# tatsuya-ogawa/metal4-raytracing

Hardware: AMD Instinct MI355X
Metric: Grays/sec (closest-hit + shadow rays traced) at 1920x1080x4spp, dragon; ms/frame (higher is better)
Workload: dtype f32; 1 GPU; c3g: glass dragon scene (configs[2]) 1920x1080x4spp, 8 bounces, one frame per step, single GPU, frames submitted back to back (overlapping frames in flight); scene=c3g, triangles=881218, width=1920, height=1080, spp=4, max_bounces=8, pipeline=wavefront, parallelism=tiles1, rays_per_frame=31537269, sort_bins=0, bvh=sah, frames_in_flight=8, animate=False

## Files before the change

metal4-raytracing_amd/csrc/rt_wavefront.hip:

```cpp
#include "rt_shade.h"
#include "rt_wavefront.h"

#include <array>
#include <utility>

namespace rt {

namespace {

__device__ __forceinline__ uint32_t lane_id() { return __builtin_amdgcn_mbcnt_hi(~0u, __builtin_amdgcn_mbcnt_lo(~0u, 0u)); }
__device__ __forceinline__ uint32_t mbcnt64(unsigned long long m) {
    return __builtin_amdgcn_mbcnt_hi((uint32_t)(m >> 32), __builtin_amdgcn_mbcnt_lo((uint32_t)m, 0u));
}

struct BlockAlloc {
    uint32_t w[kBlock / 64];
};

__device__ __forceinline__ uint32_t block_alloc(bool pred, uint32_t* counter, BlockAlloc& sh) {
    const int wave = threadIdx.x >> 6;
    unsigned long long m = __ballot(pred);
    uint32_t prefix = mbcnt64(m);
    if (lane_id() == 0) sh.w[wave] = (uint32_t)__popcll(m);
    __syncthreads();
    if (threadIdx.x == 0) {
        uint32_t c0 = sh.w[0], c1 = sh.w[1], c2 = sh.w[2], c3 = sh.w[3];
        uint32_t tot = c0 + c1 + c2 + c3;
        uint32_t b = tot ? atomicAdd(counter, tot) : 0u;
        sh.w[0] = b;
        sh.w[1] = b + c0;
        sh.w[2] = b + c0 + c1;
        sh.w[3] = b + c0 + c1 + c2;
    }
    __syncthreads();
    uint32_t r = sh.w[wave] + prefix;
    __syncthreads();
    return r;
}

struct BlockAllocOct {
    uint32_t cnt[3][8];
    uint32_t base[3][8];
};
__device__ __forceinline__ void block_alloc3_oct(const bool (&pr)[3], uint32_t oct, uint32_t* const (&ctr)[3],
                                                 BlockAllocOct& sh, uint32_t (&out)[3]) {
    if (threadIdx.x < 24) (&sh.cnt[0][0])[threadIdx.x] = 0u;
    __syncthreads();
    uint32_t rank[3] = {0u, 0u, 0u};
    #pragma unroll
    for (int i = 0; i < 3; ++i)
        if (pr[i]) rank[i] = atomicAdd(&sh.cnt[i][i ? oct : 0u], 1u);
    __syncthreads();
    if (threadIdx.x < 3) {
        const int i = threadIdx.x;
        uint32_t tot = 0, pre[8];
        #pragma unroll
        for (int o = 0; o < 8; ++o) { pre[o] = tot; tot += sh.cnt[i][o]; }
        const uint32_t b = tot ? atomicAdd(ctr[i], tot) : 0u;
        #pragma unroll
        for (int o = 0; o < 8; ++o) sh.base[i][o] = b + pre[o];
    }
    __syncthreads();
    #pragma unroll
    for (int i = 0; i < 3; ++i) out[i] = sh.base[i][i ? oct : 0u] + rank[i];
    __syncthreads();
}

__device__ __forceinline__ uint32_t block_alloc_n(uint32_t v, uint32_t* counter, BlockAlloc& sh) {
    const int wave = threadIdx.x >> 6;
    const uint32_t lane = lane_id();
    uint32_t incl = v;
    #pragma unroll
    for (int off = 1; off < 64; off <<= 1) {
        uint32_t t = __shfl_up(incl, off, 64);
        if (lane >= (uint32_t)off) incl += t;
    }
    if (lane == 63) sh.w[wave] = incl;
    __syncthreads();
    if (threadIdx.x == 0) {
        uint32_t c0 = sh.w[0], c1 = sh.w[1], c2 = sh.w[2], c3 = sh.w[3];
        uint32_t tot = c0 + c1 + c2 + c3;
        uint32_t b = tot ? atomicAdd(counter, tot) : 0u;
        sh.w[0] = b;
        sh.w[1] = b + c0;
        sh.w[2] = b + c0 + c1;
        sh.w[3] = b + c0 + c1 + c2;
    }
    __syncthreads();
    uint32_t r = sh.w[wave] + incl - v;
    __syncthreads();
    return r;
}

__device__ __forceinline__ uint32_t wave_incl_scan(uint32_t v) {
    const uint32_t lane = lane_id();
    #pragma unroll
    for (int off = 1; off < 64; off <<= 1) {
        const uint32_t t = __shfl_up(v, off, 64);
        if (lane >= (uint32_t)off) v += t;
    }
    return v;
}

__device__ __forceinline__ uint32_t compact1by1(uint32_t x) {
    x &= 0x55555555u;
    x = (x | (x >> 1)) & 0x33333333u;
    x = (x | (x >> 2)) & 0x0f0f0f0fu;
    x = (x | (x >> 4)) & 0x00ff00ffu;
    x = (x | (x >> 8)) & 0x0000ffffu;
    return x;
}


__device__ __forceinline__ uint32_t pack_state(int bounce, int tpass, int step) {
    return (uint32_t)bounce | ((uint32_t)tpass << 8) | ((uint32_t)step << 16);
}

__device__ __forceinline__ uint32_t fdiv(uint32_t n, const FastDiv& f) {
    const uint32_t t = __umulhi(f.m, n);
    return (t + ((n - t) >> f.s1)) >> f.s2;
}

__device__ __forceinline__ void own_pixel(const WfParams& Q, uint32_t i, int& px, int& py) {
    const uint32_t T = (uint32_t)Q.tile;
    const uint32_t k = fdiv(i, Q.tile_px_div), r = i - k * Q.tile_px_div.d;
    const uint32_t tid = (uint32_t)Q.rank + k * (uint32_t)Q.nranks;
    const uint32_t ty = fdiv(tid, Q.tiles_x_div), tx = tid - ty * Q.tiles_x_div.d;
    uint32_t lx, ly;
    if ((T & (T - 1)) == 0) {
        lx = compact1by1(r);
        ly = compact1by1(r >> 1);
    } else {
        lx = r % T;
        ly = r / T;
    }
    px = (int)(tx * T + lx);
    py = (int)(ty * T + ly);
}

constexpr int kCntSorted = 26;
constexpr uint32_t kNoKey = 0xffffffffu;

__device__ __forceinline__ void ts_start(const WfParams& Q, int ts) {
    if (ts >= 0 && blockIdx.x == 0 && threadIdx.x == 0) Q.W.tstamp[ts * kTsStride] = __builtin_amdgcn_s_memrealtime();
}
__device__ __forceinline__ void ts_end(const WfParams& Q, int ts, uint32_t* done) {
    if (ts < 0 || lane_id() != 0) return;
    if (atomicAdd(done, 1u) == (blockDim.x + 63u) / 64u - 1u)
        atomicMax(&Q.W.tstamp[ts * kTsStride + kTsLine * (1 + (int)(blockIdx.x % 8u))],
                  (unsigned long long)__builtin_amdgcn_s_memrealtime());
}

__device__ __forceinline__ void stat_add(const WfParams& Q, int word, uint32_t v) {
    if (blockIdx.x == 0 && threadIdx.x == 0) atomicAdd(&Q.W.counts[kWfStat + word], v);
}
__device__ __forceinline__ bool tail_mode(const WfParams& Q) {
    return Q.dev_ctl && __builtin_amdgcn_readfirstlane(Q.W.counts[cslot(kCntTailMode)]) != 0u;
}

struct ShardPrefix {
    uint32_t end[kShards];
};
__device__ __forceinline__ ShardPrefix load_prefix(const uint32_t* cnt, uint32_t cap = 0xffffffffu) {
    ShardPrefix p;
    uint32_t acc = 0;
    #pragma unroll
    for (int k = 0; k < kShards; ++k) {
        acc += min(__builtin_amdgcn_readfirstlane(cnt[cslot(k)]), cap);
        p.end[k] = acc;
    }
    return p;
}
struct QueueShards {
    uint32_t L[kShards], S[kShards];
};
__device__ __forceinline__ QueueShards load_queue(const uint32_t* counts, int q, uint32_t seg_cap) {
    QueueShards r;
    #pragma unroll
    for (int k = 0; k < kShards; ++k) {
        const uint32_t l = min(__builtin_amdgcn_readfirstlane(counts[cslot(q * kShards + k)]), seg_cap);
        r.L[k] = l;
        r.S[k] = min(__builtin_amdgcn_readfirstlane(counts[cslot(kCntBack + q * kShards + k)]), seg_cap - l);
    }
    return r;
}
__device__ __forceinline__ uint32_t queue_len(const QueueShards& qs) {
    uint32_t n = 0;
    #pragma unroll
    for (int k = 0; k < kShards; ++k) n += qs.L[k] + qs.S[k];
    return n;
}
__device__ __forceinline__ uint32_t seg_pos(uint32_t g, uint32_t l, uint32_t seg_cap) {
    return g < l ? g : seg_cap - 1u - (g - l);
}
__device__ __forceinline__ uint32_t dense_entry(const QueueShards& qs, uint32_t g, uint32_t seg_cap) {
    uint32_t ltot = 0;
    #pragma unroll
    for (int k = 0; k < kShards; ++k) ltot += qs.L[k];
    const bool back = g >= ltot;
    if (back) g -= ltot;
    uint32_t k = 0, start = 0, acc = 0;
    #pragma unroll
    for (int j = 0; j < kShards - 1; ++j) {
        acc += back ? qs.S[j] : qs.L[j];
        const bool past = g >= acc;
        k = past ? (uint32_t)(j + 1) : k;
        start = past ? acc : start;
    }
    const uint32_t i = g - start;
    return k * seg_cap + (back ? seg_cap - 1u - i : i);
}
__device__ __forceinline__ bool likely_long(const PathRegs& p) {
    return p.tpass > 0 || p.bounce < p.step;
}

__device__ __forceinline__ void init_path(const WfParams& Q, uint32_t pid, uint32_t pix, int sample, uint32_t hidx) {
    Q.W.p_accum[pid] = make_float4(0.0f, 0.0f, 0.0f, 0.0f);
    if (pid >= Q.base_paths) Q.W.p_meta[pid] = make_uint4(pix, (uint32_t)sample, 0u, hidx);
}


__device__ __forceinline__ void flush_counters(const FrameParams& P, uint32_t closest, uint32_t shadow, uint32_t paths,
                                               const TraceCounters& tc, bool count, bool overflow,
                                               bool trace_kernel = false) {
    block_flush_counters(P.counters, closest, shadow, count ? tc.nodes : 0u, count ? tc.tris : 0u, paths, overflow,
                         trace_kernel, count ? tc.lds_nodes : 0u);
}

__device__ __forceinline__ void write_pixel_outputs(const FrameParams& P, uint32_t pix, const StepResult& r, const Hit& h,
                                                    bool full) {
    if (r.primary) P.prim_hit[pix] = make_uint4(h.id, __float_as_uint(h.u), __float_as_uint(h.v), 0u);
    if (full && r.gbuf && P.gbuffer) {
        size_t plane = (size_t)P.U.width * P.U.height;
        P.gbuffer[pix] = r.g0;
        P.gbuffer[plane + pix] = r.g1;
        P.gbuffer[2 * plane + pix] = r.g2;
        P.gbuffer[3 * plane + pix] = r.g3;
    }
}

}

struct Trav {
    RaySetup R;
    float best, bu, bv, bdet;
    uint32_t best_id, g_base, g_hits, t_base, t_mask, t_valid;
    bool g_flip, hit_any;
    int sp;
};

__device__ __forceinline__ void trav_start(Trav& T, f3 o, f3 d, float tmax) {
    T.R = ray_setup(o, d);
    T.best = tmax;
    T.best_id = 0xffffffffu;
    T.bu = T.bv = 0.0f;
    T.bdet = 1.0f;
    T.g_base = 0;
    T.g_hits = 1;
    T.g_flip = false;
    T.t_mask = 0;
    T.sp = 0;
    T.hit_any = false;
}

__device__ __forceinline__ uint32_t next_node(Trav& T, int* stack, bool& overflow) {
    if (!T.g_hits) {
        --T.sp;
        const uint32_t ent = (uint32_t)stack[T.sp * kBlock];
        T.g_base = ent >> 9;
        T.g_flip = (ent >> 8) & 1u;
        T.g_hits = ent & 0xffu;
    }
    const int r = T.g_flip ? highest_bit(T.g_hits) : lowest_bit(T.g_hits);
    T.g_hits &= ~(1u << r);
    if (T.g_hits) {
        if (T.sp < kStackSize) {
            stack[T.sp * kBlock] = (int)pack_group(T.g_base, T.g_flip, T.g_hits);
            ++T.sp;
        } else {
            overflow = true;
        }
    }
    return T.g_base + (uint32_t)r;
}

template <bool COUNT>
__device__ __forceinline__ void node_step(const DevScene& S, Trav& T, int* stack, TraceCounters& tc, bool& overflow,
                                          float cull) {
    const uint32_t ni = next_node(T, stack, overflow);
    if (COUNT) tc.nodes++;
    const NodeWords w = load_node8(S.nodes8, ni);
    test_node8_words(w, T.R, 0.0f, fminf(cull, T.best), T.g_hits, T.t_mask, T.t_valid, T.g_base, T.t_base, T.g_flip);
}

template <bool COUNT>
__device__ __forceinline__ bool trav_step(const DevScene& S, Trav& T, bool any, int* stack, TraceCounters& tc,
                                          bool& overflow, float cull) {
    bool tdone = false;
    if (T.t_mask != 0u) {
        const int k0 = lowest_bit(T.t_mask);
        T.t_mask &= T.t_mask - 1u;
        const bool two = T.t_mask != 0u;
        const int k1 = two ? lowest_bit(T.t_mask) : k0;
        if (two) T.t_mask &= T.t_mask - 1u;
#ifdef RT_XP_STALE_BOUND
        const float stale_bound = fminf(cull, T.best);
#define RT_ISECT(a, b, c) intersect_rot(T.R.pre, T.R.o, a, b, c, 0.0f, stale_bound, &t, &u, &v, &dt)
#else
#define RT_ISECT(a, b, c) intersect_rot(T.R.pre, T.R.o, a, b, c, 0.0f, fminf(cull, T.best), &t, &u, &v, &dt)
#endif
        const uint32_t kz = (uint32_t)T.R.pre.kz;
        const uint32_t f0 = tri_slot(T.t_base, T.t_valid, k0) * (uint32_t)kTriFloats + kz;
        const uint32_t f1 = tri_slot(T.t_base, T.t_valid, k1) * (uint32_t)kTriFloats + kz;
        const f3 a0 = tri_window_at(S.tris, f0), a1 = tri_window_at(S.tris, f0 + 5u), a2 = tri_window_at(S.tris, f0 + 10u);
        const uint32_t ida = tri_id_at(S.tris, f0 - kz);
        const f3 b0 = tri_window_at(S.tris, f1), b1 = tri_window_at(S.tris, f1 + 5u), b2 = tri_window_at(S.tris, f1 + 10u);
        const uint32_t idb = tri_id_at(S.tris, f1 - kz);
        if (COUNT) tc.tris += two ? 2u : 1u;
        float t, u, v, dt;
        if (RT_ISECT(a0, a1, a2)) {
            const uint32_t id = ida;
            if (any) {
                T.hit_any = true;
                tdone = true;
            } else if (t < T.best || id < T.best_id) {
                T.best = t;
                T.best_id = id;
                T.bu = u;
                T.bdet = dt;
                T.bv = v;
            }
        }
        if (two && !tdone && RT_ISECT(b0, b1, b2)) {
            const uint32_t id = idb;
            if (any) {
                T.hit_any = true;
                tdone = true;
            } else if (t < T.best || id < T.best_id) {
                T.best = t;
                T.best_id = id;
                T.bu = u;
                T.bdet = dt;
                T.bv = v;
            }
        }
    }
    if (!tdone && T.t_mask == 0u && (T.g_hits != 0u || T.sp > 0)) node_step<COUNT>(S, T, stack, tc, overflow, cull);
    return tdone || (T.t_mask == 0u && T.g_hits == 0u && T.sp == 0);
#undef RT_ISECT
}

__device__ __forceinline__ uint32_t base_hidx(const FrameParams& P, int spp, uint32_t pix, int s) {
    const Uniforms& U = P.U;
    const int maxExtra = (U.enableMotionAdaptiveSampling != 0) ? max(U.motionSamplingMaxExtraSamples, 0) : 0;
    const int frameOffset = (int)U.frameIndex * (spp + maxExtra) + s;
    return (uint32_t)(int)(P.random[pix] + (unsigned)frameOffset);
}
__device__ __forceinline__ bool base_path(const FrameParams& P, const WfParams& Q, const ShadeTabs& halton, uint32_t pid,
                                          uint32_t& pix, int& s, uint32_t& hidx, f3& o, f3& d) {
    const Uniforms& U = P.U;
    const uint32_t i = fdiv(pid, Q.spp_div);
    s = (int)(pid - i * Q.spp_div.d);
    int px, py;
    own_pixel(Q, i, px, py);
    if (px >= U.width || py >= U.height) return false;
    pix = (uint32_t)py * (uint32_t)U.width + (uint32_t)px;
    hidx = base_hidx(P, Q.spp, pix, s);
    primary_ray(U, halton, px, py, (int)hidx, o, d);
    return true;
}
__device__ __forceinline__ uint3 path_meta(const FrameParams& P, const WfParams& Q, uint32_t pid) {
    if (pid >= Q.base_paths) {
        const uint4 m = Q.W.p_meta[pid];
        return make_uint3(m.x, m.y, m.w);
    }
    const uint32_t i = fdiv(pid, Q.spp_div);
    const int s = (int)(pid - i * Q.spp_div.d);
    int px, py;
    own_pixel(Q, i, px, py);
    const uint32_t pix = (uint32_t)py * (uint32_t)P.U.width + (uint32_t)px;
    return make_uint3(pix, (uint32_t)s, base_hidx(P, Q.spp, pix, s));
}
__device__ __forceinline__ void init_pixel(const FrameParams& P, uint32_t pix) {
    P.depth[pix] = 1.0e8f;
    P.motion[pix] = make_float2(0.0f, 0.0f);
    P.prim_hit[pix] = make_uint4(0xffffffffu, 0u, 0u, 0u);
    if (P.gbuffer) {
        const size_t plane = (size_t)P.U.width * P.U.height;
        const float4 z = make_float4(0, 0, 0, 0);
        P.gbuffer[pix] = z;
        P.gbuffer[plane + pix] = z;
        P.gbuffer[2 * plane + pix] = z;
        P.gbuffer[3 * plane + pix] = z;
    }
}
__global__ void __launch_bounds__(kBlock) wf_generate(DevScene S, const FrameParams* __restrict__ Pp, WfParams Q) {
    const FrameParams& P = *Pp;
    __shared__ HaltonDim lds_halton[kHaltonLds];
    __shared__ BlockAlloc ba;
    const ShadeTabs halton = load_tabs(S, lds_halton, nullptr);
    const Uniforms& U = P.U;
    const int spp = Q.spp;
    const int shard = blockIdx.x & (kShards - 1);
    float4* qout = Q.W.q[0] + 2 * (size_t)shard * Q.seg_cap;
    uint32_t n_paths = 0;
    const uint32_t total = Q.base_paths;
    if (Q.dev_ctl && blockIdx.x == 0 && threadIdx.x == 0) Q.W.counts[cslot(kCntFinishQ)] = (uint32_t)Q.finish_q;
    for (uint32_t base = blockIdx.x * kBlock; base < total; base += gridDim.x * kBlock) {
        uint32_t pid = base + threadIdx.x;
        int s = 0;
        uint32_t pix = 0, hidx = 0;
        f3 o = mk3(0, 0, 0), d = mk3(0, 0, 0);
        const bool valid = pid < total && base_path(P, Q, halton, pid, pix, s, hidx, o, d);
        if (valid) {
            init_path(Q, pid, pix, s, hidx);
            if (s == 0) init_pixel(P, pix);
            n_paths++;
        }
        bool live = valid && U.maxBounces > 0;
        uint32_t slot = block_alloc(live, &Q.W.counts[cslot(shard)], ba);
        if (live) {
            qout[2 * slot] = make_float4(o.x, o.y, o.z, __uint_as_float(pid));
            qout[2 * slot + 1] = make_float4(d.x, d.y, d.z, 0.0f);
        }
    }
    TraceCounters tc{0, 0, 0};
    flush_counters(P, 0, 0, n_paths, tc, false, false);
}

__device__ __forceinline__ float4 ld_stream(const float4* p) {
    typedef float v4f __attribute__((ext_vector_type(4)));
    const v4f v = __builtin_nontemporal_load(reinterpret_cast<const v4f*>(p));
    return make_float4(v.x, v.y, v.z, v.w);
}
template <bool FULL, bool SORTED>
__global__ void __launch_bounds__(kBlock) wf_shade(DevScene S, const FrameParams* __restrict__ Pp, WfParams Q, int cur) {
    const FrameParams& P = *Pp;
    __shared__ HaltonDim lds_halton[kHaltonLds];
    __shared__ MatRec lds_mat[kMatLds];
    __shared__ float4 lds_inst[3 * kInstLds];
    __shared__ Light lds_light[kLightLds];
    __shared__ BlockAllocOct bao;
    if (tail_mode(Q)) return;
    const ShadeTabs halton = load_tabs(S, lds_halton, lds_mat, lds_inst, lds_light, P.U.lightCount);
    const Uniforms& U = P.U;
    const int next = 1 - cur;
    const int shard = blockIdx.x & (kShards - 1);
    const QueueShards qs = load_queue(Q.W.counts, cur, Q.seg_cap);
    const float4* qin = Q.W.q[cur];
    float4* qout = Q.W.q[next] + 2 * (size_t)shard * Q.seg_cap;
    float4* qcout = Q.W.qc[next] + (size_t)shard * Q.seg_cap;
    float4* sqout = Q.W.sq + 3 * (size_t)shard * Q.seg_cap;
    f2 zero2;
    zero2.x = 0.0f;
    zero2.y = 0.0f;
    uint32_t beg = (blockIdx.x >> 3) * kBlock, end = 0, ebase = 0, lk = 0;
    const uint32_t stride = (gridDim.x >> 3) * kBlock;
    if (SORTED) {
        const uint32_t n = __builtin_amdgcn_readfirstlane(Q.W.counts[cslot(kCntSorted)]);
        beg += (uint32_t)(((uint64_t)n * (uint32_t)shard) / kShards);
        end = (uint32_t)(((uint64_t)n * (uint32_t)(shard + 1)) / kShards);
    } else {
        #pragma unroll
        for (int j = 0; j < kShards; ++j)
            if (j == shard) {
                lk = qs.L[j];
                end = qs.L[j] + qs.S[j];
            }
        ebase = (uint32_t)shard * Q.seg_cap;
    }
    for (uint32_t base = beg; base < end; base += stride) {
        uint32_t g = base + threadIdx.x;
        StepResult r;
        r.next = false;
        r.shadow = false;
        uint32_t pid = 0, nstate = 0;
        bool front = true;
        f3 rayO = mk3(0, 0, 0), rayD = mk3(0, 0, 0);
        float4 ncol = make_float4(0.0f, 0.0f, 0.0f, 0.0f);
        if (g < end) {
            float4 o, d, hv;
            size_t ce = 0;
            if (SORTED) {
                o = Q.W.sorted[4 * (size_t)g];
                d = Q.W.sorted[4 * (size_t)g + 1];
                hv = Q.W.sorted[4 * (size_t)g + 2];
                ce = 4 * (size_t)g + 3;
            } else {
                const uint32_t e = ebase + seg_pos(g, lk, Q.seg_cap);
                o = ld_stream(&qin[2 * (size_t)e]);
                d = ld_stream(&qin[2 * (size_t)e + 1]);
                hv = ld_stream(&Q.W.hits[e]);
                ce = e;
            }
            pid = __float_as_uint(o.w);
            Hit h;
            h.t = hv.x;
            h.id = __float_as_uint(hv.y);
            h.u = hv.z;
            h.v = hv.w;
            if (h.id != 0xffffffffu) {
                const uint32_t state = __float_as_uint(d.w);
                const float4 c = state == 0u ? make_float4(1.0f, 1.0f, 1.0f, 0.0f)
                                             : (SORTED ? Q.W.sorted[ce] : ld_stream(&Q.W.qc[cur][ce]));
                uint4 meta;
                if ((state & 0xffu) != 0u) {
                    meta = make_uint4(0u, 1u, state, __float_as_uint(c.w));
                } else {
                    const uint3 pm = path_meta(P, Q, pid);
                    meta = make_uint4(pm.x, pm.y, state, pm.z);
                }
                float4 a = FULL ? Q.W.p_accum[pid] : make_float4(0.0f, 0.0f, 0.0f, 0.0f);
                PathRegs p;
                p.color = mk3(c.x, c.y, c.z);
                p.accum = mk3(a.x, a.y, a.z);
                p.bounce = (int)(meta.z & 0xffu);
                p.tpass = (int)((meta.z >> 8) & 0xffu);
                p.step = (int)(meta.z >> 16);
                int sample = (int)meta.y;
                rayO = ld3(o);
                rayD = ld3(d);
                shade_step<FULL, false>(S, U, halton, (int)meta.w, sample, rayO, rayD, h, p, sample == 0 && p.step == 0,
                                 zero2, false, zero2, r);
                write_pixel_outputs(P, meta.x, r, h, FULL);
                nstate = pack_state(p.bounce, p.tpass, p.step);
                front = likely_long(p);
                ncol = make_float4(p.color.x, p.color.y, p.color.z, __uint_as_float(meta.w));
                if (__float_as_uint(p.accum.x) != __float_as_uint(a.x) || __float_as_uint(p.accum.y) != __float_as_uint(a.y) ||
                    __float_as_uint(p.accum.z) != __float_as_uint(a.z)) {
                    if (!FULL) {
                        const float4 s = Q.W.p_accum[pid];
                        p.accum = mk3(s.x + p.accum.x, s.y + p.accum.y, s.z + p.accum.z);
                    }
                    Q.W.p_accum[pid] = make_float4(p.accum.x, p.accum.y, p.accum.z, 0.0f);
                }
            }
        }
        const bool pr[3] = {r.shadow, r.next && front, r.next && !front};
        uint32_t* const ctr[3] = {&Q.W.counts[cslot(kCntShadowQ + shard)], &Q.W.counts[cslot(next * kShards + shard)],
                                  &Q.W.counts[cslot(kCntBack + next * kShards + shard)]};
        uint32_t slots[3];
        const uint32_t oct = (rayD.x < 0.0f ? 1u : 0u) | (rayD.y < 0.0f ? 2u : 0u) | (rayD.z < 0.0f ? 4u : 0u);
        block_alloc3_oct(pr, oct, ctr, bao, slots);
        const uint32_t ns = slots[0], nr = front ? slots[1] : Q.seg_cap - 1u - slots[2];
        if (r.shadow) {
            sqout[3 * (size_t)ns] = make_float4(r.so.x, r.so.y, r.so.z, __uint_as_float(pid));
            sqout[3 * (size_t)ns + 1] = make_float4(r.sd.x, r.sd.y, r.sd.z, r.stmax);
            sqout[3 * (size_t)ns + 2] = make_float4(r.contrib.x, r.contrib.y, r.contrib.z, 0.0f);
        }
        if (r.next) {
            qout[2 * (size_t)nr] = make_float4(rayO.x, rayO.y, rayO.z, __uint_as_float(pid));
            qout[2 * (size_t)nr + 1] = make_float4(rayD.x, rayD.y, rayD.z, __uint_as_float(nstate));
            qcout[nr] = ncol;
        }
    }
}

__device__ __forceinline__ void sort_range(uint32_t n, uint32_t& beg, uint32_t& end) {
    beg = (uint32_t)(((uint64_t)n * blockIdx.x) / kSortBlocks);
    end = (uint32_t)(((uint64_t)n * (blockIdx.x + 1)) / kSortBlocks);
}

__device__ __forceinline__ uint32_t sort_key(const DevScene& S, const WfParams& Q, uint32_t e, uint32_t shift) {
    const uint32_t id = __float_as_uint(Q.W.hits[e].y);
    return id == 0xffffffffu ? kNoKey : ((uint32_t)S.tri_bin[id] >> shift);
}

__global__ void __launch_bounds__(kSortThreads) wf_sort_hist(DevScene S, WfParams Q, int cur) {
    __shared__ uint32_t h[kSortMaxBins];
    if (tail_mode(Q)) return;
    const uint32_t shift = __builtin_ctz(kSortMaxBins) - __builtin_ctz(Q.sort_bins);
    const uint32_t K = Q.sort_bins;
    const QueueShards qs = load_queue(Q.W.counts, cur, Q.seg_cap);
    for (uint32_t k = threadIdx.x; k < K; k += kSortThreads) h[k] = 0;
    __syncthreads();
    uint32_t beg, end;
    sort_range(queue_len(qs), beg, end);
    for (uint32_t g = beg + threadIdx.x; g < end; g += kSortThreads) {
        const uint32_t k = sort_key(S, Q, dense_entry(qs, g, Q.seg_cap), shift);
        if (k != kNoKey) atomicAdd(&h[k], 1u);
    }
    __syncthreads();
    for (uint32_t k = threadIdx.x; k < K; k += kSortThreads) Q.W.sort_table[(size_t)k * kSortBlocks + blockIdx.x] = h[k];
}

__global__ void __launch_bounds__(kSortBlocks) wf_sort_rowscan(WfParams Q) {
    __shared__ uint32_t w[kSortBlocks / 64];
    if (tail_mode(Q)) return;
    uint32_t* row = Q.W.sort_table + (size_t)blockIdx.x * kSortBlocks;
    const uint32_t v = row[threadIdx.x];
    const uint32_t incl = wave_incl_scan(v);
    const int wave = threadIdx.x >> 6;
    if (lane_id() == 63) w[wave] = incl;
    __syncthreads();
    uint32_t base = 0;
    for (int i = 0; i < wave; ++i) base += w[i];
    row[threadIdx.x] = base + incl - v;
    if (threadIdx.x == kSortBlocks - 1) Q.W.sort_total[blockIdx.x] = base + incl;
}

__global__ void __launch_bounds__(kSortThreads) wf_sort_scatter(DevScene S, WfParams Q, int cur) {
    __shared__ uint32_t off[kSortMaxBins];
    if (tail_mode(Q)) return;
    const uint32_t shift = __builtin_ctz(kSortMaxBins) - __builtin_ctz(Q.sort_bins);
    __shared__ uint32_t w[kSortThreads / 64];
    const uint32_t K = Q.sort_bins, per = K / kSortThreads;
    const QueueShards qs = load_queue(Q.W.counts, cur, Q.seg_cap);
    uint32_t loc[kSortMaxBins / kSortThreads];
    uint32_t s = 0;
    for (uint32_t i = 0; i < per; ++i) {
        loc[i] = s;
        s += Q.W.sort_total[threadIdx.x * per + i];
    }
    const uint32_t incl = wave_incl_scan(s);
    const int wave = threadIdx.x >> 6;
    if (lane_id() == 63) w[wave] = incl;
    __syncthreads();
    uint32_t base = 0;
    for (int i = 0; i < wave; ++i) base += w[i];
    const uint32_t excl = base + incl - s;
    for (uint32_t i = 0; i < per; ++i) {
        const uint32_t k = threadIdx.x * per + i;
        off[k] = excl + loc[i] + Q.W.sort_table[(size_t)k * kSortBlocks + blockIdx.x];
    }
    if (blockIdx.x == 0 && threadIdx.x == kSortThreads - 1) Q.W.counts[cslot(kCntSorted)] = excl + s;
    __syncthreads();
    const float4* qin = Q.W.q[cur];
    uint32_t beg, end;
    sort_range(queue_len(qs), beg, end);
    for (uint32_t g = beg + threadIdx.x; g < end; g += kSortThreads) {
        const uint32_t e = dense_entry(qs, g, Q.seg_cap);
        const float4 hv = Q.W.hits[e];
        const uint32_t id = __float_as_uint(hv.y);
        if (id == 0xffffffffu) continue;
        const uint32_t pos = atomicAdd(&off[(uint32_t)S.tri_bin[id] >> shift], 1u);
        const float4 o = qin[2 * (size_t)e], d = qin[2 * (size_t)e + 1];
        Q.W.sorted[4 * (size_t)pos] = o;
        Q.W.sorted[4 * (size_t)pos + 1] = d;
        Q.W.sorted[4 * (size_t)pos + 2] = hv;
        if (__float_as_uint(d.w) != 0u) Q.W.sorted[4 * (size_t)pos + 3] = Q.W.qc[cur][e];
    }
}

__device__ __forceinline__ void connect_flush(const WfParams& Q, const float4* qin, uint32_t* pend, uint32_t& npend) {
    __builtin_amdgcn_fence(__ATOMIC_SEQ_CST, "wavefront");
    __builtin_amdgcn_wave_barrier();
    const uint32_t lane = lane_id();
    if (lane < npend) {
        const uint32_t e = pend[lane];
        const float4 o4 = qin[3 * (size_t)e];
        const float4 c = qin[3 * (size_t)e + 2];
        const uint32_t pid = __float_as_uint(o4.w);
        const float4 a = Q.W.p_accum[pid];
        Q.W.p_accum[pid] = make_float4(a.x + c.x, a.y + c.y, a.z + c.z, 0.0f);
    }
    __builtin_amdgcn_fence(__ATOMIC_SEQ_CST, "wavefront");
    __builtin_amdgcn_wave_barrier();
    npend = 0;
}

template <bool ANY, bool COUNT>
#ifndef RT_EXTEND_WAVES
#define RT_EXTEND_WAVES 8
#endif
__global__ void __launch_bounds__(kBlock) __attribute__((amdgpu_waves_per_eu(ANY ? 8 : RT_EXTEND_WAVES, ANY ? 8 : RT_EXTEND_WAVES)))
wf_trace(DevScene S, const FrameParams* __restrict__ Pp, WfParams Q, int cur, int ts) {
    const FrameParams& P = *Pp;
    __shared__ int lds_stack[kStackSize * kBlock];
    int* stack = &lds_stack[threadIdx.x];
    if (Q.dev_ctl) {
        const bool tm = tail_mode(Q);
        if (ANY) {
            if (tm) return;
        } else {
            if (tm || queue_len(load_queue(Q.W.counts, cur, Q.seg_cap)) < Q.tail) {
                if (!tm && blockIdx.x == 0 && threadIdx.x == 0) {
                    Q.W.counts[cslot(kCntTailMode)] = 1u;
                    Q.W.counts[cslot(kCntFinishQ)] = (uint32_t)cur;
                }
                return;
            }
        }
    }
    __shared__ uint32_t ts_done;
    if (threadIdx.x == 0) ts_done = 0u;
    ts_start(Q, ts);
    __syncthreads();
    const uint32_t n = ANY ? load_prefix(Q.W.counts + cslot(kCntShadowQ)).end[kShards - 1]
                           : queue_len(load_queue(Q.W.counts, cur, Q.seg_cap));
    if (Q.dev_ctl) {
        stat_add(Q, kStatTraceRays, n);
        stat_add(Q, kStatTraceLaunches, 1u);
        if (!ANY) {
            stat_add(Q, kStatRounds, 1u);
            stat_add(Q, kStatExtendRays, n);
        }
    }
    if (!ANY && blockIdx.x == 0 && threadIdx.x < 3 * kShards) {
        const int next = 1 - cur;
        const uint32_t k = threadIdx.x & (kShards - 1), part = threadIdx.x / kShards;
        Q.W.counts[cslot(part == 0 ? next * kShards + k : part == 1 ? kCntShadowQ + k : kCntBack + next * kShards + k)] = 0;
    }
    if (blockIdx.x == 0 && threadIdx.x < kShards)
        Q.W.counts[cslot((ANY ? kCntChunkExtend : kCntChunkConnect) + threadIdx.x)] = 0;
    const float4* qin = ANY ? Q.W.sq : Q.W.q[cur];
    const int qstride = ANY ? 3 : 2;
    const uint32_t xcd = blockIdx.x & 7u;
    uint32_t* const chunk_ctr = Q.W.counts + cslot((ANY ? kCntChunkConnect : kCntChunkExtend) + (int)xcd);
    uint32_t xl, xend;
    if (ANY) {
        xl = xend = min(__builtin_amdgcn_readfirstlane(Q.W.counts[cslot(kCntShadowQ + (int)xcd)]), Q.seg_cap);
    } else {
        xl = min(__builtin_amdgcn_readfirstlane(Q.W.counts[cslot(cur * kShards + (int)xcd)]), Q.seg_cap);
        xend = xl + min(__builtin_amdgcn_readfirstlane(Q.W.counts[cslot(kCntBack + cur * kShards + (int)xcd)]),
                        Q.seg_cap - xl);
    }
    const uint32_t xbeg = 0, ebase = xcd * Q.seg_cap;
    uint32_t wnext = 0, wend = 0;
    bool exhausted = false;

    TraceCounters tc{0, 0, 0};
    bool overflow = false;
    uint32_t rays = 0;
    bool active = false;
    uint32_t e = 0;
    Trav T;
    trav_start(T, mk3(0, 0, 0), mk3(1, 0, 0), 0.0f);
    uint32_t steps = 0;
    __shared__ uint32_t lds_pend_all[ANY ? kBlock : 1];
    uint32_t* const lds_pend = &lds_pend_all[ANY ? (threadIdx.x & ~63u) : 0u];
    uint32_t npend = 0;

    while (true) {
        const unsigned long long idle = __ballot(!active);
        const bool refill = __popcll(idle) >= Q.refill_min || idle == ~0ull;
        if (wnext >= wend && !exhausted && refill) {
            uint32_t base = 0;
            if (lane_id() == 0) base = atomicAdd(chunk_ctr, (uint32_t)Q.chunk);
            base = xbeg + __builtin_amdgcn_readfirstlane(base);
            if (base >= xend) {
                exhausted = true;
            } else {
                wnext = base;
                wend = min(base + (uint32_t)Q.chunk, xend);
            }
        }
        if (idle != 0ull && wnext < wend && refill) {
            if (!active) {
                uint32_t g = wnext + mbcnt64(idle);
                if (g < wend) {
                    e = ebase + (ANY ? g : seg_pos(g, xl, Q.seg_cap));
                    float4 o4 = qin[(size_t)qstride * e];
                    float4 d4 = qin[(size_t)qstride * e + 1];
                    trav_start(T, ld3(o4), ld3(d4), ANY ? d4.w : INFINITY);
                    active = true;
                    rays++;
                    if (COUNT) steps = 0;
                }
            }
            wnext += (uint32_t)__popcll(idle);
        }
        if (__ballot(active) == 0ull) {
            if (ANY) connect_flush(Q, qin, lds_pend, npend);
            break;
        }
        bool acc = false;
        if (active) {
            if (COUNT) ++steps;
            if (trav_step<COUNT>(S, T, ANY, stack, tc, overflow, T.best)) {
                active = false;
                if (COUNT && Q.diag) {
                    atomicAdd(&Q.W.counts[kWfDiagSteps + (ANY ? 32 : 0) + (31 - __builtin_clz(steps))], 1u);
                    atomicMax(&Q.W.counts[kWfDiagSteps + 64 + (ANY ? 1 : 0)], steps);
                }
                if (ANY) acc = !T.hit_any;
                else Q.W.hits[e] = make_float4(T.best, __uint_as_float(T.best_id), T.bu / T.bdet, T.bv / T.bdet);
            }
        }
        if (ANY) {
            const unsigned long long m = __ballot(acc);
            if (m != 0ull) {
                const uint32_t k = (uint32_t)__popcll(m);
                if (npend + k > 64u) connect_flush(Q, qin, lds_pend, npend);
                if (acc) lds_pend[npend + mbcnt64(m)] = e;
                npend += k;
            }
        }
    }
    ts_end(Q, ts, &ts_done);
    flush_counters(P, ANY ? 0 : rays, ANY ? rays : 0, 0, tc, COUNT, overflow, true);
}

template <bool COUNT, bool FULL, bool TEAM>
__global__ void __launch_bounds__(kBlock) __attribute__((amdgpu_waves_per_eu(4, 4)))
wf_finish_step(DevScene S, const FrameParams* __restrict__ Pp, WfParams Q, int cur, int ts) {
    const FrameParams& P = *Pp;
    if (cur < 0) cur = (int)__builtin_amdgcn_readfirstlane(Q.W.counts[cslot(kCntFinishQ)]);
    __shared__ int lds_stack[kStackSize * kBlock];
    __shared__ HaltonDim lds_halton[kHaltonLds];
    __shared__ MatRec lds_mat[kMatLds];
    __shared__ float4 lds_inst[3 * kInstLds];
    __shared__ Light lds_light[kLightLds];
    __shared__ float lds_sray[6][kBlock];
    int* stack = &lds_stack[threadIdx.x];
    __shared__ uint32_t ts_done;
    if (threadIdx.x == 0) ts_done = 0u;
    ts_start(Q, ts);
    const ShadeTabs halton = load_tabs(S, lds_halton, lds_mat, lds_inst, lds_light, P.U.lightCount);
    const Uniforms& U = P.U;
    const QueueShards qs = load_queue(Q.W.counts, cur, Q.seg_cap);
    const uint32_t n = queue_len(qs);
    if (Q.dev_ctl) stat_add(Q, kStatFinish, 1u);
    if (Q.dev_ctl && n > 0) stat_add(Q, kStatRounds, 1u);
    const float4* qin = Q.W.q[cur];
    const uint32_t kChunk = (uint32_t)Q.fchunk;
    constexpr int kIdle = 0, kClosest = 1, kShadow = 2, kReady = 3;
    TraceCounters tc{0, 0, 0};
    bool overflow = false;
    uint32_t n_closest = 0, n_shadow = 0;
    f2 zero2;
    zero2.x = 0.0f;
    zero2.y = 0.0f;
    uint32_t wnext = 0, wend = 0;
    bool exhausted = false;
    int mode = kIdle;
    uint32_t pid = 0;
    uint4 meta = make_uint4(0, 0, 0, 0);
    PathRegs p;
    p.color = p.accum = mk3(0, 0, 0);
    p.bounce = p.tpass = p.step = 0;
    f3 rayO = mk3(0, 0, 0), rayD = mk3(0, 0, 0), contrib = mk3(0, 0, 0);
    bool next = false;
    Trav T;
    trav_start(T, mk3(0, 0, 0), mk3(1, 0, 0), 0.0f);
    uint32_t segs = 0, max_segs = 0, iters = 0;
    const uint64_t t_start = Q.diag ? __builtin_amdgcn_s_memrealtime() : 0;
    __shared__ uint32_t diag_x[kBlock / 64][3];
#define RT_DX diag_x[__builtin_amdgcn_readfirstlane(threadIdx.x) / 64u]
    if (Q.diag && lane_id() == 0) RT_DX[0] = RT_DX[1] = RT_DX[2] = 0xffffffffu;
    uint64_t t_shade = 0;
    uint32_t n_pass = 0, n_shaded = 0;
    auto end_path = [&]() {
        Q.W.p_accum[pid] = make_float4(p.accum.x, p.accum.y, p.accum.z, 0.0f);
        if (Q.diag > 1) {
            const uint32_t b0 = min(meta.z & 0xffu, 8u), tp0 = (meta.z >> 8) & 0xffu;
            atomicAdd(&Q.W.counts[kWfDiagLen + ((tp0 ? 9u : 0u) + b0) * 32u + min(segs, 31u)], 1u);
        }
        mode = kIdle;
        max_segs = max(max_segs, segs);
        segs = 0;
    };

    auto shade_hit = [&](StepResult& r) {
        Hit h;
        h.t = T.best;
        h.id = T.best_id;
        h.u = T.bu / T.bdet;
        h.v = T.bv / T.bdet;
        const int sample = (int)meta.y;
        shade_step<FULL, false>(S, U, halton, (int)meta.w, sample, rayO, rayD, h, p, sample == 0 && p.step == 0, zero2,
                                false, zero2, r);
        write_pixel_outputs(P, meta.x, r, h, FULL);
        next = r.next;
    };

    while (true) {
        const unsigned long long idle = __ballot(mode == kIdle);
        const bool refill = __popcll(idle) >= Q.refill_min || idle == ~0ull;
        if (wnext >= wend && !exhausted && refill) {
            uint32_t base = 0;
            if (lane_id() == 0) base = atomicAdd(Q.W.counts + cslot(kCntChunkFinish + (int)(blockIdx.x & 7u)), 1u);
            base = ((__builtin_amdgcn_readfirstlane(base) << 3) | (blockIdx.x & 7u)) * kChunk;
            if (base >= n) {
                exhausted = true;
                if (Q.diag && lane_id() == 0) {
                    RT_DX[0] = iters;
                    RT_DX[1] = (uint32_t)(__builtin_amdgcn_s_memrealtime() - t_start);
                    RT_DX[2] = 0;
                }
            } else {
                wnext = base;
                wend = min(base + kChunk, n);
            }
        }
        if (idle != 0ull && wnext < wend && refill) {
            if (mode == kIdle) {
                const uint32_t g = wnext + mbcnt64(idle);
                if (g < wend) {
                    const uint32_t e = dense_entry(qs, g, Q.seg_cap);
                    const float4* src = qin + 2 * (size_t)e;
                    const float4 o = ld_stream(&src[0]);
                    const float4 d = ld_stream(&src[1]);
                    pid = __float_as_uint(o.w);
                    const uint32_t state = __float_as_uint(d.w);
                    const float4 c = state == 0u ? make_float4(1.0f, 1.0f, 1.0f, 0.0f)
                                     : ld_stream(&Q.W.qc[cur][e]);
                    if ((state & 0xffu) != 0u) {
                        meta = make_uint4(0u, 1u, state, __float_as_uint(c.w));
                    } else {
                        const uint3 pm = path_meta(P, Q, pid);
                        meta = make_uint4(pm.x, pm.y, state, pm.z);
                    }
                    const float4 a = Q.W.p_accum[pid];
                    p.color = mk3(c.x, c.y, c.z);
                    p.accum = mk3(a.x, a.y, a.z);
                    p.bounce = (int)(meta.z & 0xffu);
                    p.tpass = (int)((meta.z >> 8) & 0xffu);
                    p.step = (int)(meta.z >> 16);
                    rayO = ld3(o);
                    rayD = ld3(d);
                    trav_start(T, rayO, rayD, INFINITY);
                    mode = kClosest;
                    n_closest++;
                    segs++;
                }
            }
            wnext += (uint32_t)__popcll(idle);
        }
        const unsigned long long active = __ballot(mode != kIdle);
        if (active == 0ull) break;
        if (TEAM && exhausted && __popcll(active) * Q.team <= 64) break;
        ++iters;
        if (Q.diag && exhausted && lane_id() == 0) RT_DX[2] += (uint32_t)__popcll(active);

        if (mode == kClosest || mode == kShadow) {
            const bool any = mode == kShadow;
            if (trav_step<COUNT>(S, T, any, stack, tc, overflow, T.best)) {
                if (any) {
                    if (!T.hit_any) p.accum = p.accum + contrib;
                    if (next) {
                        trav_start(T, rayO, rayD, INFINITY);
                        mode = kClosest;
                        n_closest++;
                        segs++;
                    } else {
                        end_path();
                    }
                } else if (T.best_id == 0xffffffffu) {
                    end_path();
                } else {
                    mode = kReady;
                }
            }
        }

        const unsigned long long ready = __ballot(mode == kReady);
        int shade_thr = exhausted ? Q.shade_min_x : Q.shade_min;
        if (shade_thr < 0) shade_thr = max(1, -shade_thr * __popcll(__ballot(mode != kIdle)) / 100);
        if (ready != 0ull && (__popcll(ready) >= shade_thr || __ballot(mode == kClosest || mode == kShadow) == 0ull)) {
            const uint64_t ts0 = Q.diag ? __builtin_amdgcn_s_memrealtime() : 0;
            if (Q.diag) {
                ++n_pass;
                n_shaded += (uint32_t)__popcll(ready);
            }
            if (mode == kReady) {
                StepResult r;
                shade_hit(r);
                if (r.shadow) {
                    contrib = r.contrib;
                    trav_start(T, r.so, r.sd, r.stmax);
                    lds_sray[0][threadIdx.x] = r.so.x;
                    lds_sray[1][threadIdx.x] = r.so.y;
                    lds_sray[2][threadIdx.x] = r.so.z;
                    lds_sray[3][threadIdx.x] = r.sd.x;
                    lds_sray[4][threadIdx.x] = r.sd.y;
                    lds_sray[5][threadIdx.x] = r.sd.z;
                    mode = kShadow;
                    n_shadow++;
                } else if (r.next) {
                    trav_start(T, rayO, rayD, INFINITY);
                    mode = kClosest;
                    n_closest++;
                    segs++;
                } else {
                    end_path();
                }
            }
            if (mode == kShadow) {
                T.R = ray_setup(mk3(lds_sray[0][threadIdx.x], lds_sray[1][threadIdx.x], lds_sray[2][threadIdx.x]),
                                mk3(lds_sray[3][threadIdx.x], lds_sray[4][threadIdx.x], lds_sray[5][threadIdx.x]));
            } else {
                T.R = ray_setup(rayO, rayD);
            }
            if (Q.diag) t_shade += __builtin_amdgcn_s_memrealtime() - ts0;
        }

    }

    if (TEAM && __ballot(mode != kIdle) != 0ull) {
        const int TM = Q.team;
        if (mode == kReady) {
            StepResult r;
            shade_hit(r);
            if (r.shadow) {
                contrib = r.contrib;
                trav_start(T, r.so, r.sd, r.stmax);
                lds_sray[0][threadIdx.x] = r.so.x;
                lds_sray[1][threadIdx.x] = r.so.y;
                lds_sray[2][threadIdx.x] = r.so.z;
                lds_sray[3][threadIdx.x] = r.sd.x;
                lds_sray[4][threadIdx.x] = r.sd.y;
                lds_sray[5][threadIdx.x] = r.sd.z;
                mode = kShadow;
                n_shadow++;
            } else if (r.next) {
                mode = kClosest;
                n_closest++;
                segs++;
            } else {
                end_path();
            }
        }
        const unsigned long long busy = __ballot(mode != kIdle);
        const int lane = (int)lane_id(), j = lane & (TM - 1), lead = lane - j, rk = lane / TM;
        const int nb = __popcll(busy);
        int src = lane;
        {
            unsigned long long b = busy;
            for (int k = 0; b; ++k) {
                const int l = __builtin_ctzll(b);
                b &= b - 1ull;
                if (j == 0 && rk == k) src = l;
            }
        }
        const bool leader = j == 0 && rk < nb;
        auto mvu = [&](uint32_t v) { return (uint32_t)__shfl((int)v, src); };
        auto mvf = [&](float v) { return __shfl(v, src); };
        auto mv3 = [&](f3 v) { return mk3(mvf(v.x), mvf(v.y), mvf(v.z)); };
        const uint32_t sbase = threadIdx.x & ~63u;
        {
            float sr[6];
            #pragma unroll
            for (int c = 0; c < 6; ++c) sr[c] = lds_sray[c][sbase + src];
            #pragma unroll
            for (int c = 0; c < 6; ++c) lds_sray[c][threadIdx.x] = sr[c];
        }
        __shared__ float lds_tx[4][kBlock];
        {
            const float t_src = mvf(T.best);
            const f3 c_src = mv3(contrib);
            lds_tx[0][threadIdx.x] = t_src;
            lds_tx[1][threadIdx.x] = c_src.x;
            lds_tx[2][threadIdx.x] = c_src.y;
            lds_tx[3][threadIdx.x] = c_src.z;
        }
        pid = mvu(pid);
        meta = make_uint4(mvu(meta.x), mvu(meta.y), mvu(meta.z), mvu(meta.w));
        p.color = mv3(p.color);
        p.accum = mv3(p.accum);
        p.bounce = (int)mvu((uint32_t)p.bounce);
        p.step = (int)mvu((uint32_t)p.step);
        p.tpass = (int)mvu((uint32_t)p.tpass);
        rayO = mv3(rayO);
        rayD = mv3(rayD);
        next = mvu(next ? 1u : 0u) != 0u;
        segs = mvu(segs);
        const int src_mode = (int)mvu((uint32_t)mode);
        mode = leader ? src_mode : kIdle;
        bool fresh = leader;
        float cull = INFINITY;
        while (true) {
            const int lmode = __shfl(mode, lead);
            if (__ballot(lmode != kIdle) == 0ull) break;
            const bool team_on = lmode == kClosest || lmode == kShadow, any = lmode == kShadow;
            if (__shfl((int)fresh, lead) != 0 && team_on) {
                f3 o, d;
                float tmax;
                if (any) {
                    const uint32_t ls = sbase + (uint32_t)lead;
                    o = mk3(lds_sray[0][ls], lds_sray[1][ls], lds_sray[2][ls]);
                    d = mk3(lds_sray[3][ls], lds_sray[4][ls], lds_sray[5][ls]);
                    tmax = lds_tx[0][ls];
                } else {
                    o = mk3(__shfl(rayO.x, lead), __shfl(rayO.y, lead), __shfl(rayO.z, lead));
                    d = mk3(__shfl(rayD.x, lead), __shfl(rayD.y, lead), __shfl(rayD.z, lead));
                    tmax = INFINITY;
                }
                trav_start(T, o, d, tmax);
                if (j != 0) T.g_hits = 0;
                cull = tmax;
            }
            fresh = false;
            if (team_on && !(T.t_mask == 0u && T.g_hits == 0u && T.sp == 0))
                (void)trav_step<COUNT>(S, T, any, stack, tc, overflow, cull);
            int hit = (any && T.hit_any) ? 1 : 0;
            float bt = T.best;
            for (int k = 1; k < TM; k <<= 1) {
                hit |= __shfl_xor(hit, k);
                bt = fminf(bt, __shfl_xor(bt, k));
            }
            if (team_on && !any) cull = bt;
            if (hit) {
                T.t_mask = 0u;
                T.g_hits = 0u;
                T.sp = 0;
            }
            for (int k = 1; k < TM; ++k) {
                const bool idle_m = team_on && T.t_mask == 0u && T.g_hits == 0u && T.sp == 0;
                const bool give = team_on && (__popc(T.g_hits) >= 2 || T.sp > 0);
                const bool p_idle = __shfl_xor((int)idle_m, k) != 0, p_give = __shfl_xor((int)give, k) != 0;
                uint32_t pay = 0u;
                if (give && p_idle) {
                    if (__popc(T.g_hits) >= 2) {
                        uint32_t keep = 0u, rest = T.g_hits;
                        for (int c = __popc(T.g_hits) - __popc(T.g_hits) / 2; c > 0; --c) {
                            const int b = T.g_flip ? highest_bit(rest) : lowest_bit(rest);
                            keep |= 1u << b;
                            rest &= ~(1u << b);
                        }
                        pay = pack_group(T.g_base, T.g_flip, rest);
                        T.g_hits = keep;
                    } else {
                        --T.sp;
                        pay = (uint32_t)stack[T.sp * kBlock];
                    }
                }
                const uint32_t got = (uint32_t)__shfl_xor((int)pay, k);
                if (idle_m && p_give) {
                    T.g_base = got >> 9;
                    T.g_flip = (got >> 8) & 1u;
                    T.g_hits = got & 0xffu;
                }
            }
            int work = (team_on && !(T.t_mask == 0u && T.g_hits == 0u && T.sp == 0)) ? 1 : 0;
            for (int k = 1; k < TM; k <<= 1) work |= __shfl_xor(work, k);
            if (team_on && !work) {
                if (!any) {
                    float t = T.best, bu = T.bu, bv = T.bv, bd = T.bdet;
                    uint32_t id = T.best_id;
                    for (int k = 1; k < TM; k <<= 1) {
                        const float t2 = __shfl_xor(t, k), u2 = __shfl_xor(bu, k), v2 = __shfl_xor(bv, k),
                                    d2 = __shfl_xor(bd, k);
                        const uint32_t id2 = (uint32_t)__shfl_xor((int)id, k);
                        if (t2 < t || (t2 == t && id2 < id)) {
                            t = t2;
                            id = id2;
                            bu = u2;
                            bv = v2;
                            bd = d2;
                        }
                    }
                    T.best = t;
                    T.best_id = id;
                    T.bu = bu;
                    T.bv = bv;
                    T.bdet = bd;
                }
                if (j == 0) {
                    if (any) {
                        if (!hit)
                            p.accum = p.accum + mk3(lds_tx[1][threadIdx.x], lds_tx[2][threadIdx.x], lds_tx[3][threadIdx.x]);
                        if (next) {
                            mode = kClosest;
                            n_closest++;
                            segs++;
                            fresh = true;
                        } else {
                            end_path();
                        }
                    } else if (T.best_id == 0xffffffffu) {
                        end_path();
                    } else {
                        mode = kReady;
                    }
                }
            }
            if (mode == kReady) {
                StepResult r;
                shade_hit(r);
                if (r.shadow) {
                    lds_tx[1][threadIdx.x] = r.contrib.x;
                    lds_tx[2][threadIdx.x] = r.contrib.y;
                    lds_tx[3][threadIdx.x] = r.contrib.z;
                    lds_sray[0][threadIdx.x] = r.so.x;
                    lds_sray[1][threadIdx.x] = r.so.y;
                    lds_sray[2][threadIdx.x] = r.so.z;
                    lds_sray[3][threadIdx.x] = r.sd.x;
                    lds_sray[4][threadIdx.x] = r.sd.y;
                    lds_sray[5][threadIdx.x] = r.sd.z;
                    lds_tx[0][threadIdx.x] = r.stmax;
                    mode = kShadow;
                    n_shadow++;
                    fresh = true;
                } else if (r.next) {
                    mode = kClosest;
                    n_closest++;
                    segs++;
                    fresh = true;
                } else {
                    end_path();
                }
            }
        }
    }

    if (Q.diag) {
        const uint32_t dt = (uint32_t)(__builtin_amdgcn_s_memrealtime() - t_start);
        if (lane_id() == 0) {
            const uint32_t* dx = RT_DX;
            const bool x = dx[0] != 0xffffffffu;
            const uint32_t it_x = x ? dx[0] : iters, t_x = x ? dx[1] : dt;
            atomicAdd(&Q.W.counts[kWfStat + kStatDiagItPre], it_x);
            atomicAdd(&Q.W.counts[kWfStat + kStatDiagItPost], iters - it_x);
            atomicAdd(&Q.W.counts[kWfStat + kStatDiagTPre], t_x);
            atomicAdd(&Q.W.counts[kWfStat + kStatDiagTPost], dt - t_x);
            atomicAdd(&Q.W.counts[kWfStat + kStatDiagLanesPost], x ? dx[2] : 0u);
            atomicAdd(&Q.W.counts[kWfDiagExh + min(t_x / 5000u, 63u)], 1u);
            atomicAdd(&Q.W.counts[kWfStat + kStatDiagShadeT], (uint32_t)t_shade);
            atomicAdd(&Q.W.counts[kWfStat + kStatDiagTotalT], dt);
            atomicAdd(&Q.W.counts[kWfStat + kStatDiagPasses], n_pass);
            atomicAdd(&Q.W.counts[kWfStat + kStatDiagShaded], n_shaded);
        }
        for (int off = 32; off > 0; off >>= 1) max_segs = max(max_segs, (uint32_t)__shfl_xor((int)max_segs, off, 64));
        if (lane_id() == 0) {
            atomicMax(&Q.W.counts[cslot(kCntDiagSegs)], max_segs);
            atomicMax(&Q.W.counts[cslot(kCntDiagIters)], iters);
            atomicMax(&Q.W.counts[cslot(kCntDiagTime)], dt);
            atomicAdd(&Q.W.counts[kWfDiagHist + min(dt / 5000u, 63u)], 1u);
        }
    }
#undef RT_DX
    ts_end(Q, ts, &ts_done);
    flush_counters(P, n_closest, n_shadow, 0, tc, COUNT, overflow);
}

__global__ void __launch_bounds__(kBlock) wf_extra(DevScene S, const FrameParams* __restrict__ Pp, WfParams Q, int qidx) {
    const FrameParams& P = *Pp;
    __shared__ HaltonDim lds_halton[kHaltonLds];
    const ShadeTabs halton = load_tabs(S, lds_halton, nullptr);
    const Uniforms& U = P.U;
    const int maxExtra = (U.enableMotionAdaptiveSampling != 0) ? max(U.motionSamplingMaxExtraSamples, 0) : 0;
    const int stride = Q.spp + maxExtra;
    const int shard = blockIdx.x & (kShards - 1);
    float4* qout = Q.W.q[qidx] + 2 * (size_t)shard * Q.seg_cap;
    __shared__ BlockAlloc ba;
    const uint32_t i = blockIdx.x * kBlock + threadIdx.x;
    int px = 0, py = 0, e = 0;
    uint32_t pix = 0;
    if (i < Q.own_pixels) {
        own_pixel(Q, i, px, py);
        if (px < U.width && py < U.height) {
            pix = (uint32_t)py * (uint32_t)U.width + (uint32_t)px;
            float2 mv2 = P.motion[pix], pm2 = P.motion_prev[pix];
            f2 mv, pm;
            mv.x = mv2.x;
            mv.y = mv2.y;
            pm.x = pm2.x;
            pm.y = pm2.y;
            e = extra_samples(U, maxExtra, mv, pm);
        }
    }
    const uint32_t start = block_alloc_n((uint32_t)e, &Q.W.counts[cslot(kCntExtra)], ba);
    const uint32_t slot0 =
        block_alloc_n(U.maxBounces > 0 ? (uint32_t)e : 0u, &Q.W.counts[cslot(qidx * kShards + shard)], ba);
    if (e > 0) {
        const uint32_t offset = P.random[pix];
        for (int j = 0; j < e; ++j) {
            int s = Q.spp + j;
            uint32_t pid = Q.base_paths + start + (uint32_t)j;
            int hidx = (int)(offset + (unsigned)((int)U.frameIndex * stride + s));
            init_path(Q, pid, pix, s, (uint32_t)hidx);
            f3 o, d;
            primary_ray(U, halton, px, py, hidx, o, d);
            if (U.maxBounces > 0) {
                const uint32_t slot = slot0 + (uint32_t)j;
                qout[2 * (size_t)slot] = make_float4(o.x, o.y, o.z, __uint_as_float(pid));
                qout[2 * (size_t)slot + 1] = make_float4(d.x, d.y, d.z, 0.0f);
            }
        }
    }
    if (i < Q.own_pixels) Q.W.px_extra[i] = make_uint2(start, (uint32_t)e);
    TraceCounters tc{0, 0, 0};
    flush_counters(P, 0, 0, (uint32_t)e, tc, false, false);
}

__global__ void __launch_bounds__(kBlock) wf_motion(DevScene S, const FrameParams* __restrict__ Pp, WfParams Q) {
    const FrameParams& P = *Pp;
    const Uniforms& U = P.U;
    const uint32_t i = blockIdx.x * kBlock + threadIdx.x;
    if (i >= Q.own_pixels) return;
    int px, py;
    own_pixel(Q, i, px, py);
    if (px >= U.width || py >= U.height) return;
    const size_t pix = (size_t)py * U.width + px;
    const uint4 ph = P.prim_hit[pix];
    if (ph.x == 0xffffffffu) return;
    float depth;
    f2 mv;
    primary_outputs(S, U, ph.x, __uint_as_float(ph.y), __uint_as_float(ph.z), depth, mv);
    P.depth[pix] = depth;
    P.motion[pix] = make_float2(mv.x, mv.y);
}

__global__ void __launch_bounds__(kBlock) wf_resolve(DevScene S, const FrameParams* __restrict__ Pp, WfParams Q, int with_extra) {
    const FrameParams& P = *Pp;
    const Uniforms& U = P.U;
    uint32_t i = blockIdx.x * kBlock + threadIdx.x;
    if (i >= Q.own_pixels) return;
    int px, py;
    own_pixel(Q, i, px, py);
    if (px >= U.width || py >= U.height) return;
    size_t pix = (size_t)py * U.width + px;
    f3 total = mk3(0.0f, 0.0f, 0.0f);
    for (int s = 0; s < Q.spp; ++s) {
        float4 a = Q.W.p_accum[(size_t)i * Q.spp + s];
        total = total + mk3(a.x, a.y, a.z);
    }
    int nsamp = Q.spp;
    if (with_extra) {
        uint2 ex = Q.W.px_extra[i];
        for (uint32_t j = 0; j < ex.y; ++j) {
            float4 a = Q.W.p_accum[Q.base_paths + ex.x + j];
            total = total + mk3(a.x, a.y, a.z);
        }
        nsamp += (int)ex.y;
    }
    float2 mv2 = P.motion[pix], pm2 = P.motion_prev[pix];
    f2 mv, pm;
    mv.x = mv2.x;
    mv.y = mv2.y;
    pm.x = pm2.x;
    pm.y = pm2.y;
    f3 c = resolve_pixel(U, total, nsamp, mv, pm, P.accum_in, pix);
    P.accum_out[pix] = make_float4(c.x, c.y, c.z, 1.0f);
}

template <typename K>
static unsigned resident_grid(K kernel, int fallback_per_cu) {
    int dev = 0, cus = 256, per = 0;
    if (hipGetDevice(&dev) == hipSuccess) (void)hipDeviceGetAttribute(&cus, hipDeviceAttributeMultiprocessorCount, dev);
    if (hipOccupancyMaxActiveBlocksPerMultiprocessor(&per, kernel, kBlock, 0) != hipSuccess || per < 1)
        per = fallback_per_cu;
    return (unsigned)(cus * per);
}

template <bool COUNT, bool FULL, bool SORTED, bool TEAM>
static WfKernels kernel_set() {
    WfKernels K = {wf_trace<false, COUNT>, wf_trace<true, COUNT>, wf_finish_step<COUNT, FULL, TEAM>,
                   wf_shade<FULL, SORTED>, wf_extra, wf_resolve, wf_generate, wf_motion,
                   wf_sort_hist, wf_sort_scatter, wf_sort_rowscan, 0u, 0u};
    K.finish_resident = resident_grid(K.finish, 2);
    return K;
}

template <size_t... I>
static std::array<WfKernels, 16> kernel_table(std::index_sequence<I...>) {
    std::array<WfKernels, 16> t = {{kernel_set<(I >> 3) & 1, (I >> 2) & 1, (I >> 1) & 1, I & 1>()...}};
    const unsigned trace = resident_grid(t[0].extend, 4);
    for (WfKernels& k : t) k.trace_resident = trace;
    return t;
}

const WfKernels& wf_kernels(bool count, bool full, bool sorted, bool team) {
    static const std::array<WfKernels, 16> table = kernel_table(std::make_index_sequence<16>());
    return table[(count ? 8 : 0) | (full ? 4 : 0) | (sorted ? 2 : 0) | (team ? 1 : 0)];
}

}
```

Measured before the change: 10.35 Grays/s.

## Compact hit rays into shared-memory ring before shading in unsorted path

In the unsorted shade kernel, each block now reads hit records first, ballots on whether each one is a hit, and compacts hit entries (index and hit data) into a shared-memory ring buffer. Shading then runs on full blocks of compacted hits, which removes lanes left idle by misses and avoids loading ray origin and direction for missed entries. The cost is extra __syncthreads per fill, LDS usage for the ring, and a more complex loop structure. Misses no longer pass through the shading body in this path, so any per-miss work done there (such as environment contribution) would be skipped if it existed.

Result: faster. 10.66 Grays/s (median of 6 runs) (+3.0%).

```diff
diff --git a/metal4-raytracing_amd/csrc/rt_wavefront.hip b/metal4-raytracing_amd/csrc/rt_wavefront.hip
--- a/metal4-raytracing_amd/csrc/rt_wavefront.hip
+++ b/metal4-raytracing_amd/csrc/rt_wavefront.hip
@@ -469,8 +469,60 @@
             }
         ebase = (uint32_t)shard * Q.seg_cap;
     }
-    for (uint32_t base = beg; base < end; base += stride) {
+    constexpr uint32_t kRing = 2 * kBlock;
+    __shared__ uint32_t ring_e[SORTED ? 1 : kRing];
+    __shared__ float4 ring_h[SORTED ? 1 : kRing];
+    __shared__ uint32_t ring_w[2][kBlock / 64];
+    uint32_t head = 0, pending = 0, fills = 0;
+    uint32_t base = beg;
+    while (true) {
         uint32_t g = base + threadIdx.x;
+        bool valid;
+        uint32_t slot = 0;
+        if (SORTED) {
+            if (base >= end) break;
+            valid = g < end;
+            base += stride;
+        } else {
+            while (pending < (uint32_t)kBlock && base < end) {
+                g = base + threadIdx.x;
+                uint32_t e = 0;
+                float4 hv = make_float4(0.0f, 0.0f, 0.0f, 0.0f);
+                bool hit = false;
+                if (g < end) {
+                    e = ebase + seg_pos(g, lk, Q.seg_cap);
+                    hv = ld_stream(&Q.W.hits[e]);
+                    hit = __float_as_uint(hv.y) != 0xffffffffu;
+                }
+                const unsigned long long m = __ballot(hit);
+                uint32_t* const w = ring_w[fills & 1u];
+                const uint32_t wave = __builtin_amdgcn_readfirstlane(threadIdx.x >> 6);
+                if (lane_id() == 0) w[wave] = (uint32_t)__popcll(m);
+                __syncthreads();
+                uint32_t off = 0, tot = 0;
+                #pragma unroll
+                for (uint32_t j = 0; j < (uint32_t)(kBlock / 64); ++j) {
+                    const uint32_t c = w[j];
+                    off += j < wave ? c : 0u;
+                    tot += c;
+                }
+                if (hit) {
+                    const uint32_t s = (head + pending + off + mbcnt64(m)) & (kRing - 1u);
+                    ring_e[s] = e;
+                    ring_h[s] = hv;
+                }
+                pending += __builtin_amdgcn_readfirstlane(tot);
+                ++fills;
+                base += stride;
+            }
+            if (pending == 0u) break;
+            __syncthreads();
+            const uint32_t n = min(pending, (uint32_t)kBlock);
+            valid = threadIdx.x < n;
+            slot = (head + threadIdx.x) & (kRing - 1u);
+            head = (head + n) & (kRing - 1u);
+            pending -= n;
+        }
         StepResult r;
         r.next = false;
         r.shadow = false;
@@ -478,7 +530,7 @@
         bool front = true;
         f3 rayO = mk3(0, 0, 0), rayD = mk3(0, 0, 0);
         float4 ncol = make_float4(0.0f, 0.0f, 0.0f, 0.0f);
-        if (g < end) {
+        if (valid) {
             float4 o, d, hv;
             size_t ce = 0;
             if (SORTED) {
@@ -487,10 +539,10 @@
                 hv = Q.W.sorted[4 * (size_t)g + 2];
                 ce = 4 * (size_t)g + 3;
             } else {
-                const uint32_t e = ebase + seg_pos(g, lk, Q.seg_cap);
+                const uint32_t e = ring_e[slot];
+                hv = ring_h[slot];
                 o = ld_stream(&qin[2 * (size_t)e]);
                 d = ld_stream(&qin[2 * (size_t)e + 1]);
-                hv = ld_stream(&Q.W.hits[e]);
                 ce = e;
             }
             pid = __float_as_uint(o.w);
@@ -499,7 +551,7 @@
             h.id = __float_as_uint(hv.y);
             h.u = hv.z;
             h.v = hv.w;
-            if (h.id != 0xffffffffu) {
+            if (!SORTED || h.id != 0xffffffffu) {
                 const uint32_t state = __float_as_uint(d.w);
                 const float4 c = state == 0u ? make_float4(1.0f, 1.0f, 1.0f, 0.0f)
                                              : (SORTED ? Q.W.sorted[ce] : ld_stream(&Q.W.qc[cur][ce]));
```
